# cram9030/continuum-robot

Hardware: AMD Instinct MI355X
Metric: beam-element-steps/s (higher is better)
Workload: dtype f64

## Files before the change

### continuum-robot_amd/csrc/crb_lean.h

```cpp
#pragma once
#include <hip/hip_runtime.h>

#include "crb_blocked.h"
#include "crb_generic.h"

namespace crb {

template <typename T>
struct LeanRec {
    static constexpr int N = sizeof(T) == 8 ? 10 : 12;
    static constexpr int V = 16 / sizeof(T);
};
template <typename T>
__host__ __device__ constexpr size_t lean_lds_bytes(int NT, int lognw) {
    return sizeof(T) * (size_t(NT + 1) * LeanRec<T>::N * (lognw == 1 ? 2 : 1) +
                        (sizeof(T) == 4 ? 4 : 3) * size_t(NT + 1) * size_t(lognw > 1 ? lognw - 1 : 0));
}

__device__ __forceinline__ double dpp_from_lower(double x) {
    int lo = __double2loint(x), hi = __double2hiint(x);
    lo = __builtin_amdgcn_mov_dpp(lo, 0x138, 0xf, 0xf, true);
    hi = __builtin_amdgcn_mov_dpp(hi, 0x138, 0xf, 0xf, true);
    return __hiloint2double(hi, lo);
}
__device__ __forceinline__ double dpp_from_higher(double x) {
    int lo = __double2loint(x), hi = __double2hiint(x);
    lo = __builtin_amdgcn_mov_dpp(lo, 0x130, 0xf, 0xf, true);
    hi = __builtin_amdgcn_mov_dpp(hi, 0x130, 0xf, 0xf, true);
    return __hiloint2double(hi, lo);
}
__device__ __forceinline__ float dpp_from_lower(float x) {
    return __int_as_float(__builtin_amdgcn_mov_dpp(__float_as_int(x), 0x138, 0xf, 0xf, true));
}
__device__ __forceinline__ float dpp_from_higher(float x) {
    return __int_as_float(__builtin_amdgcn_mov_dpp(__float_as_int(x), 0x130, 0xf, 0xf, true));
}
constexpr int LEAN_DPP_MAX = 4;
constexpr int P_FORCE = 0, P_XCHG = 2, P_L1 = -1, P_TAIL = 1, P_FIN = -1;
constexpr int P32_L1 = 3, P32_TAIL = 3, P32_FIN = 0;
#define CRB_SETPRIO(v) do { if ((v) >= 0) __builtin_amdgcn_s_setprio((v) < 0 ? 0 : (v)); } while (0)
template <typename T, int D>
__device__ __forceinline__ T lane_lower(T x, int lane) {
    if (D <= LEAN_DPP_MAX) {
#pragma unroll
        for (int i = 0; i < D; ++i) x = dpp_from_lower(x);
        return x;
    }
    return __shfl(x, lane - D, 64);
}
template <typename T, int D>
__device__ __forceinline__ T lane_higher(T x, int lane) {
    if (D <= LEAN_DPP_MAX) {
#pragma unroll
        for (int i = 0; i < D; ++i) x = dpp_from_higher(x);
        return x;
    }
    return __shfl(x, lane + D, 64);
}

template <typename T, int LV, int LOGNW, bool ISOLATE = false, bool RECB = false>
__device__ __forceinline__ void lean_reduce_tail(const SolveCoef<T, LV>& cf, T* ldsB, int t, int lane, int j, int S,
                                                 bool valid, T r[3], T a[3]) {
    constexpr int NW = 1 << LOGNW, NT = 64 << LOGNW, NULLT = NT;
    auto thread_of = [](int jj) { return ((jj & (NW - 1)) << 6) | (jj >> LOGNW); };
    T rlo[3], rhi[3];
#pragma unroll
    for (int l = 1; l < LV; ++l) {
        if (l < LOGNW) {
            if (l == 1) CRB_SETPRIO(sizeof(T) == 4 ? P32_L1 : P_L1);
            const int st = 1 << l;
            const int tl = (valid && j - st >= 0) ? thread_of(j - st) : NULLT;
            const int th = (valid && j + st < S) ? thread_of(j + st) : NULLT;
            if constexpr (RECB) {
                typedef T rec4 __attribute__((ext_vector_type(4)));
                rec4* buf = reinterpret_cast<rec4*>(ldsB) + size_t(l - 1) * (NT + 1);
                buf[t] = rec4{r[0], r[1], r[2], T(0)};
                __syncthreads();
                const rec4 lo = buf[tl], hi = buf[th];
#pragma unroll
                for (int c = 0; c < 3; ++c) { rlo[c] = lo[c]; rhi[c] = hi[c]; }
            } else {
                T* buf = ldsB + size_t(l - 1) * 3 * (NT + 1);
                buf[t] = r[0]; buf[(NT + 1) + t] = r[1]; buf[2 * (NT + 1) + t] = r[2];
                __syncthreads();
#pragma unroll
                for (int c = 0; c < 3; ++c) { rlo[c] = buf[c * (NT + 1) + tl]; rhi[c] = buf[c * (NT + 1) + th]; }
            }
        } else {
            if (l == LOGNW) CRB_SETPRIO(sizeof(T) == 4 ? P32_TAIL : P_TAIL);
#pragma unroll
            for (int c = 0; c < 3; ++c) {
                switch (l - LOGNW) {
                    case 0: rlo[c] = lane_lower<T, 1>(r[c], lane); rhi[c] = lane_higher<T, 1>(r[c], lane); break;
                    case 1: rlo[c] = lane_lower<T, 2>(r[c], lane); rhi[c] = lane_higher<T, 2>(r[c], lane); break;
                    case 2: rlo[c] = lane_lower<T, 4>(r[c], lane); rhi[c] = lane_higher<T, 4>(r[c], lane); break;
                    case 3: rlo[c] = lane_lower<T, 8>(r[c], lane); rhi[c] = lane_higher<T, 8>(r[c], lane); break;
                    case 4: rlo[c] = lane_lower<T, 16>(r[c], lane); rhi[c] = lane_higher<T, 16>(r[c], lane); break;
                    default: rlo[c] = lane_lower<T, 32>(r[c], lane); rhi[c] = lane_higher<T, 32>(r[c], lane); break;
                }
            }
            if (ISOLATE) {
                const int st = 1 << l;
                const bool lo_ok = valid && j - st >= 0, hi_ok = valid && j + st < S;
#pragma unroll
                for (int c = 0; c < 3; ++c) { rlo[c] = lo_ok ? rlo[c] : T(0); rhi[c] = hi_ok ? rhi[c] : T(0); }
            }
        }
        pcr_apply_level<T>(cf.lv[l], rlo, rhi, r);
    }
    CRB_SETPRIO(sizeof(T) == 4 ? P32_FIN : P_FIN);
    pcr_apply_final<T>(cf.fin, r, a);
}

template <typename T, int LV, int LOGNW, int EM>
__device__ __forceinline__ void lean_rhs(const ElemCoef<T>& ec, T dragc, bool corrected, const SolveCoef<T, LV>& cf, T* lds3, int t,
                                         int lane, int j, int S, bool valid, const T sq[3], const T sv[3], const T uadd[3], T a[3]) {
    constexpr int NW = 1 << LOGNW, NT = 64 << LOGNW, NULLT = NT;
    T* const ldsQ = lds3;
    T* const ldsA = lds3 + 3 * size_t(NT + 1);
    T* const ldsB = lds3 + 9 * size_t(NT + 1);
    auto thread_of = [](int jj) { return ((jj & (NW - 1)) << 6) | (jj >> LOGNW); };
    const int t_l1 = (valid && j >= 1) ? thread_of(j - 1) : NULLT;
    const int t_r1 = (valid && j + 1 < S) ? thread_of(j + 1) : NULLT;
    const int t_r2 = (valid && j + 2 < S) ? thread_of(j + 2) : NULLT;
    T qL[3];
    if (LOGNW == 0) {
#pragma unroll
        for (int c = 0; c < 3; ++c) qL[c] = lane_lower<T, 1>(sq[c], lane);
    } else {
#pragma unroll
        for (int c = 0; c < 3; ++c) ldsQ[size_t(c) * (NT + 1) + t] = sq[c];
        __syncthreads();
#pragma unroll
        for (int c = 0; c < 3; ++c) qL[c] = ldsQ[size_t(c) * (NT + 1) + t_l1];
    }
    T fl[3], fr[3];
    if (EM == EM_NONLINEAR) elem_force_nonlinear<T>(ec.c, qL, sq, false, fl, fr);
    else if (EM == EM_LINEAR) elem_force_linear<T>(ec.c, qL, sq, fl, fr);
    else elem_force<T>(ec, qL, sq, corrected, fl, fr);
    T pp[3];
#pragma unroll
    for (int c = 0; c < 3; ++c) pp[c] = uadd[c] - fr[c];
    pp[1] += drag_force<T>(dragc, sv[1]);
    T r[3], rlo[3], rhi[3];
    if (LOGNW == 0) {
#pragma unroll
        for (int c = 0; c < 3; ++c) {
            r[c] = pp[c] - lane_higher<T, 1>(fl[c], lane);
            rlo[c] = lane_lower<T, 1>(r[c], lane);
            rhi[c] = lane_higher<T, 1>(r[c], lane);
        }
    } else {
        auto col = [&](int k, int th) -> T& { return ldsA[size_t(k) * (NT + 1) + th]; };
#pragma unroll
        for (int c = 0; c < 3; ++c) { col(c, t) = pp[c]; col(3 + c, t) = fl[c]; }
        __syncthreads();
#pragma unroll
        for (int c = 0; c < 3; ++c) {
            rlo[c] = col(c, t_l1) - fl[c];
            r[c] = pp[c] - col(3 + c, t_r1);
            rhi[c] = col(c, t_r1) - col(3 + c, t_r2);
        }
    }
    pcr_apply_level<T>(cf.lv[0], rlo, rhi, r);
    lean_reduce_tail<T, LV, LOGNW>(cf, ldsB, t, lane, j, S, valid, r, a);
}

constexpr int BLK_STRIP_PAD = 4;
constexpr int BLK_STRIP_W = BLK_STRIP_PAD + BLK_LANES + BLK_STRIP_PAD;
__host__ __device__ constexpr size_t blk_lds_bytes(int ls) {
    return size_t(blk_sep_vals(ls) + 1) / 2 * 2 * BLK_LANES * sizeof(double) + size_t(4) * 3 * BLK_STRIP_W * sizeof(double);
}
template <typename T, int LS, int EM, typename KPT>
__device__ __forceinline__ void lean_blocked_body(KPT kp) {
    static_assert(sizeof(T) == 8, "the blocked stepper is fp64");
    static_assert(LS == 3 && (1 << (LS - 1)) == BLK_STRIP_PAD, "the strip carries the third separator level, stride 4");
    constexpr int NP = BLK_NPL, NV = blk_sep_vals(LS), NV2 = (NV + 1) / 2;
    constexpr bool REGROUP = EM == EM_NONLINEAR && !CRB_LITERAL_POLY;
#if defined(__HIP_DEVICE_COMPILE__)
    typedef const __attribute__((address_space(4))) SlotConst<T>* CS;
#define CRB_BFRESH(ptr) asm volatile("" : "+s"(ptr))
#else
    typedef const SlotConst<T>* CS;
#define CRB_BFRESH(ptr) (void)(ptr)
#endif
    typedef T rec4 __attribute__((ext_vector_type(4)));
    typedef T pair2 __attribute__((ext_vector_type(2)));
    KParams<T> p = *(const KParams<T>*)(kp);
    extern __shared__ __attribute__((aligned(16))) unsigned char crb_smem[];
    pair2* const sepL = reinterpret_cast<pair2*>(crb_smem);
    T* const strips = reinterpret_cast<T*>(sepL + NV2 * 64);
    const int t = threadIdx.x, lane = t & 63;
    const int wave = __builtin_amdgcn_readfirstlane(t >> 6);
    {
        const T* src = p.blocked + BU_N;
        for (int i = t; i < NV2 * 64; i += 256) {
            const int v = 2 * (i >> 6), l = i & 63;
            sepL[i] = pair2{src[size_t(v) * 64 + l], v + 1 < NV ? src[size_t(v + 1) * 64 + l] : T(0)};
        }
        for (int i = t; i < 4 * 3 * BLK_STRIP_W; i += 256) {
            const int k = i % BLK_STRIP_W;
            if (k < BLK_STRIP_PAD || k >= BLK_STRIP_PAD + BLK_LANES) strips[i] = T(0);
        }
    }
#if defined(__HIP_DEVICE_COMPILE__)
    typedef volatile __attribute__((address_space(3))) T* SP;
#else
    typedef volatile T* SP;
#endif
    const SP strip = (SP)(strips + wave * 3 * BLK_STRIP_W + BLK_STRIP_PAD + lane);
    T tab[BLK_TAB_REGS];
#pragma unroll
    for (int i = 0; i < BLK_TAB_REGS; ++i) tab[i] = p.blocked[blk_tab_index(i, lane)];
    const T cD2[3] = {blk_bc_copy<BU_D2>(tab), blk_bc_copy<BU_D2 + 2>(tab), blk_bc_copy<BU_D2 + 4>(tab)};
    const T cD1[3] = {blk_bc_copy<BU_U1>(tab), blk_bc_copy<BU_D1 + 2>(tab), blk_bc_copy<BU_D1 + 4>(tab)};
    const T cD0[3] = {blk_bc_copy<BU_U0>(tab), blk_bc_copy<BU_D0 + 2>(tab), blk_bc_copy<BU_D0 + 4>(tab)};
    __syncthreads();
    const int n_groups = (p.B + 3) / 4;
    for (int grp = blockIdx.x; grp < n_groups; grp += gridDim.x) {
        CRB_BFRESH(kp);
        p = *(const KParams<T>*)(kp);
        const int beam = grp * 4 + wave;
        if (beam >= p.B) continue;
        const size_t plane = size_t(p.n_node) * 4;
        const size_t xoff = size_t(beam) * 2 * plane + size_t(NP * lane + p.off) * 4;
        T xq[NP][3], xv[NP][3];
#pragma unroll
        for (int k = 0; k < NP; ++k) {
            const rec4 a = *reinterpret_cast<const rec4*>(p.x + xoff + 4 * k), b = *reinterpret_cast<const rec4*>(p.x + xoff + plane + 4 * k);
#pragma unroll
            for (int c = 0; c < 3; ++c) { xq[k][c] = a[c]; xv[k][c] = b[c]; }
        }
        T amp = T(0);
        int kimp = -1;
        if (p.amp) {
            const int js = p.imp_node_b ? p.imp_node_b[beam] - p.off : p.imp_slot;
            if (js >= 0 && js < BLK_S) {
                kimp = js & (NP - 1);
                if (lane == js / NP) amp = p.amp[beam];
            }
        }
        T qL[3];
#pragma unroll
        for (int c = 0; c < 3; ++c) qL[c] = dpp_from_lower(xq[NP - 1][c]);
        const T dt = T(p.dt), hdt = T(0.5 * p.dt), dt6 = T(p.dt / 6.0);
        double tc = p.t0;
        T accq[NP][3], accv[NP][3], sq[NP][3], sv[NP][3];
        for (int step = 0; step < p.n_steps; ++step) {
            double t_half, t_full;
            {
                KPT ks = kp;
                CRB_BFRESH(ks);
                const double hstep = (*(const KParams<T>*)(ks)).dt;
                t_half = __dadd_rn(tc, 0.5 * hstep);
                t_full = __dadd_rn(tc, hstep);
            }
#pragma unroll
            for (int k = 0; k < NP; ++k)
#pragma unroll
                for (int c = 0; c < 3; ++c) { sq[k][c] = xq[k][c]; sv[k][c] = xv[k][c]; }
#pragma unroll
            for (int s = 0; s < 4; ++s) {
                KPT ks = kp;
                CRB_BFRESH(ks);
                const KParams<T>& q = *(const KParams<T>*)(ks);
                const double ts = (s == 0) ? tc : ((s == 3) ? t_full : t_half);
                const bool imp_on = ts < q.duration;
                const T w = (s == 0 || s == 3) ? T(1) : T(2);
                const T cs = (s == 2) ? dt : hdt;
                const CS SC = (CS)q.slot;
                T ec[6];
#pragma unroll
                for (int i = 0; i < 6; ++i) ec[i] = SC->elem.c[i];
                const T drag_all = SC->drag;
                const T dragc = (q.flags & 1u) ? drag_all : T(0);
                T qn3[3], qLn[3];
#pragma unroll
                for (int k = 0; k < NP; ++k)
#pragma unroll
                    for (int c = 0; c < 3; ++c) accq[k][c] = (s == 0) ? sv[k][c] : accq[k][c] + w * sv[k][c];
#pragma unroll
                for (int c = 0; c < 3; ++c) {
                    qn3[c] = (s == 3) ? (xq[NP - 1][c] + dt6 * accq[NP - 1][c]) : (xq[NP - 1][c] + cs * sv[NP - 1][c]);
                    qLn[c] = dpp_from_lower(qn3[c]);
                }
                CRB_SETPRIO(P_FORCE);
                T fl[NP][3], r[NP][3];
                T fr[NP][3];
                T f2[NP], cW[NP];
#pragma unroll
                for (int k = 0; k < NP; ++k) {
                    if constexpr (REGROUP) {
                        const ElemForceRegrouped<T> e = elem_force_nonlinear_regrouped<T>(ec, k ? sq[k - 1] : qL, sq[k]);
                        f2[k] = e.f2; cW[k] = ec[1] * e.W;
                        fl[k][1] = e.f3; fr[k][1] = -e.f3; fl[k][2] = e.m_left; fr[k][2] = e.m_right;
                    } else if (EM == EM_NONLINEAR) elem_force_nonlinear<T>(ec, k ? sq[k - 1] : qL, sq[k], false, fl[k], fr[k]);
                    else elem_force_linear<T>(ec, k ? sq[k - 1] : qL, sq[k], fl[k], fr[k]);
                }
                if constexpr (REGROUP) {
                    fl[0][0] = cW[0] - f2[0];
#pragma unroll
                    for (int k = 0; k + 1 < NP; ++k) fr[k][0] = f2[k] - f2[k + 1];
                    fr[NP - 1][0] = dpp_from_higher(fl[0][0]);
                }
                {
                    const int kon = imp_on ? kimp : -1, dof = q.imp_dof;
#if defined(__HIP_DEVICE_COMPILE__)
#pragma unroll
                    for (int k = 0; k < NP; ++k)
                        asm volatile(
                            "s_cmp_lg_u32 %[kon], %[k]\n\t"
                            "s_cbranch_scc1 2f\n\t"
                            "s_cmp_lg_u32 %[dof], 0\n\t"
                            "s_cbranch_scc1 0f\n\t"
                            "v_add_f64 %[f0], %[f0], -%[amp]\n"
                            "0:\n\t"
                            "s_cmp_lg_u32 %[dof], 1\n\t"
                            "s_cbranch_scc1 1f\n\t"
                            "v_add_f64 %[f1], %[f1], -%[amp]\n"
                            "1:\n\t"
                            "s_cmp_lg_u32 %[dof], 2\n\t"
                            "s_cbranch_scc1 2f\n\t"
                            "v_add_f64 %[f2], %[f2], -%[amp]\n"
                            "2:"
                            : [f0] "+v"(fr[k][0]), [f1] "+v"(fr[k][1]), [f2] "+v"(fr[k][2])
                            : [kon] "s"(kon), [dof] "s"(dof), [amp] "v"(amp), [k] "n"(k)
                            : "scc");
#else
                    for (int k = 0; k < NP; ++k)
                        for (int c = 0; c < 3; ++c) fr[k][c] -= (kon == k && c == dof) ? amp : T(0);
#endif
                }
                CRB_SETPRIO(P_TAIL);
#pragma unroll
                for (int c = 0; c < 3; ++c) {
                    if (REGROUP && c == 0) {
#pragma unroll
                        for (int k = 0; k < NP; ++k) r[k][0] = (k + 1 < NP) ? (-fr[k][0] - cW[k + 1]) : (-f2[k] - fr[k][0]);
                        continue;
                    }
                    const T flR = dpp_from_higher(fl[0][c]);
#pragma unroll
                    for (int k = 0; k < NP; ++k) {
                        T h = -fr[k][c];
                        if (c == 1) h += drag_force<T>(dragc, sv[k][1]);
                        r[k][c] = h - ((k + 1 < NP) ? fl[k + 1][c] : flR);
                    }
                }
                T y[3][3], z1[3], z2[3], g[3], y0R[3];
                int li = lane;
                T cf0[PCR_LEVEL_VALS];
                asm volatile("" : "+v"(li) : "v"(r[0][0]));
#pragma unroll
                for (int i = 0; i < PCR_LEVEL_VALS; i += 2) {
                    const pair2 e = sepL[(i / 2) * 64 + li];
                    cf0[i] = e[0]; cf0[i + 1] = e[1];
                }
#pragma unroll
                for (int c = 0; c < 3; ++c) { z1[c] = r[1][c]; z2[c] = r[2][c]; g[c] = r[NP - 1][c]; }
                blk_bc_sub_mul<BU_L1>(tab, r[0], z1);
                blk_bc_sub_mul<BU_L2>(tab, z1, z2);
                y[2][0] = cD2[0] * z2[0];
                y[2][1] = cD2[1] * z2[2]; blk_bc_fma<BU_D2 + 1>(tab, z2[1], y[2][1]);
                y[2][2] = cD2[2] * z2[2]; blk_bc_fma<BU_D2 + 3>(tab, z2[1], y[2][2]);
                y[1][0] = -(cD1[0] * y[2][0]); blk_bc_fma<BU_D1>(tab, z1[0], y[1][0]);
                y[1][1] = cD1[1] * z1[2]; blk_bc_fma<BU_D1 + 1>(tab, z1[1], y[1][1]);
                y[1][2] = cD1[2] * z1[2]; blk_bc_fma<BU_D1 + 3>(tab, z1[1], y[1][2]);
                blk_bc_fnma<BU_U1 + 1>(tab, y[2][1], y[1][1]); blk_bc_fnma<BU_U1 + 2>(tab, y[2][2], y[1][1]);
                blk_bc_fnma<BU_U1 + 3>(tab, y[2][1], y[1][2]); blk_bc_fnma<BU_U1 + 4>(tab, y[2][2], y[1][2]);
                y[0][0] = -(cD0[0] * y[1][0]); blk_bc_fma<BU_D0>(tab, r[0][0], y[0][0]);
                y[0][1] = cD0[1] * r[0][2]; blk_bc_fma<BU_D0 + 1>(tab, r[0][1], y[0][1]);
                y[0][2] = cD0[2] * r[0][2]; blk_bc_fma<BU_D0 + 3>(tab, r[0][1], y[0][2]);
                blk_bc_fnma<BU_U0 + 1>(tab, y[1][1], y[0][1]); blk_bc_fnma<BU_U0 + 2>(tab, y[1][2], y[0][1]);
                blk_bc_fnma<BU_U0 + 3>(tab, y[1][1], y[0][2]); blk_bc_fnma<BU_U0 + 4>(tab, y[1][2], y[0][2]);
#pragma unroll
                for (int c = 0; c < 3; ++c) y0R[c] = dpp_from_higher(y[0][c]);
                blk_bc_sub_mul<BU_AS>(tab, y[2], g);
                blk_bc_sub_mul<BU_CS>(tab, y0R, g);
#pragma unroll
                for (int l = 0; l < LS; ++l) {
                    asm volatile("" : "+v"(li) : "v"(g[0]));
                    T cf[PCR_LEVEL_VALS];
#pragma unroll
                    for (int i = 0; i < PCR_LEVEL_VALS; i += 2) {
                        const int v = l * PCR_LEVEL_VALS + i;
                        if (l == 0) { cf[i] = cf0[i]; cf[i + 1] = cf0[i + 1]; continue; }
                        const pair2 e = sepL[(v / 2) * 64 + li];
                        cf[i] = e[0]; cf[i + 1] = e[1];
                    }
                    T glo[3], ghi[3];
                    if (l == 2) {
#pragma unroll
                        for (int c = 0; c < 3; ++c) strip[c * BLK_STRIP_W] = g[c];
#pragma unroll
                        for (int c = 0; c < 3; ++c) { glo[c] = strip[c * BLK_STRIP_W - 4]; ghi[c] = strip[c * BLK_STRIP_W + 4]; }
                    } else if (l == 1) {
#pragma unroll
                        for (int c = 0; c < 3; ++c) { glo[c] = lane_lower<T, 2>(g[c], lane); ghi[c] = lane_higher<T, 2>(g[c], lane); }
                    } else {
#pragma unroll
                        for (int c = 0; c < 3; ++c) { glo[c] = lane_lower<T, 1>(g[c], lane); ghi[c] = lane_higher<T, 1>(g[c], lane); }
                    }
                    pcr_apply_level<T>(cf, glo, ghi, g);
                }
                asm volatile("" : "+v"(li) : "v"(g[0]));
                T fin[6], xs[3], xsL[3];
#pragma unroll
                for (int i = 0; i < 6; i += 2) {
                    const int v = LS * PCR_LEVEL_VALS + i;
                    const pair2 e = sepL[(v / 2) * 64 + li];
                    fin[i] = e[0]; fin[i + 1] = e[1];
                }
                pcr_apply_final<T>(fin, g, xs);
#pragma unroll
                for (int c = 0; c < 3; ++c) xsL[c] = dpp_from_lower(xs[c]);
                T a[NP][3];
#pragma unroll
                for (int k = 0; k < NP - 1; ++k)
#pragma unroll
                    for (int c = 0; c < 3; ++c) a[k][c] = y[k][c];
                static_assert(NP == 4, "three interior nodes, written out: the table offsets are template arguments");
                blk_bc_sub_mul<BU_WL>(tab, xsL, a[0]);
                blk_bc_sub_mul<BU_WR>(tab, xs, a[0]);
                blk_bc_sub_mul<BU_WL + BLK_PACK>(tab, xsL, a[1]);
                blk_bc_sub_mul<BU_WR + BLK_PACK>(tab, xs, a[1]);
                blk_bc_sub_mul<BU_WL + 2 * BLK_PACK>(tab, xsL, a[2]);
                blk_bc_sub_mul<BU_WR + 2 * BLK_PACK>(tab, xs, a[2]);
#pragma unroll
                for (int c = 0; c < 3; ++c) a[NP - 1][c] = xs[c];
#pragma unroll
                for (int k = 0; k < NP; ++k)
#pragma unroll
                    for (int c = 0; c < 3; ++c) {
                        accv[k][c] = (s == 0) ? a[k][c] : accv[k][c] + w * a[k][c];
                        if (k == NP - 1) sq[k][c] = qn3[c];
                        else sq[k][c] = (s == 3) ? (xq[k][c] + dt6 * accq[k][c]) : (xq[k][c] + cs * sv[k][c]);
                        sv[k][c] = (s == 3) ? (xv[k][c] + dt6 * accv[k][c]) : (xv[k][c] + cs * a[k][c]);
                    }
#pragma unroll
                for (int c = 0; c < 3; ++c) qL[c] = qLn[c];
            }
#pragma unroll
            for (int k = 0; k < NP; ++k)
#pragma unroll
                for (int c = 0; c < 3; ++c) { xq[k][c] = sq[k][c]; xv[k][c] = sv[k][c]; }
            tc = t_full;
            KPT kr_ = kp;
            CRB_BFRESH(kr_);
            const KParams<T>& pr = *(const KParams<T>*)(kr_);
            if (pr.rec_out && (step + 1) % pr.rec_every == 0) {
                const size_t kr = size_t((step + 1) / pr.rec_every - 1);
                if (pr.rec_slot == REC_ALL_SLOTS) {
                    T* snap = pr.rec_out + kr * size_t(pr.B) * 2 * plane + xoff;
#pragma unroll
                    for (int k = 0; k < NP; ++k) {
                        *reinterpret_cast<rec4*>(snap + 4 * k) = rec4{xq[k][0], xq[k][1], xq[k][2], T(0)};
                        *reinterpret_cast<rec4*>(snap + plane + 4 * k) = rec4{xv[k][0], xv[k][1], xv[k][2], T(0)};
                    }
                } else if (pr.rec_slot >= 0 && lane == pr.rec_slot / NP) {
                    const int kk = pr.rec_slot & (NP - 1);
                    T val = xq[0][0];
#pragma unroll
                    for (int k = 0; k < NP; ++k)
#pragma unroll
                        for (int c = 0; c < 6; ++c)
                            val = (k == kk && c == pr.rec_comp) ? (c < 3 ? xq[k][c] : xv[k][c - 3]) : val;
                    pr.rec_out[size_t(beam) * pr.rec_n + kr] = val;
                }
            }
        }
        CRB_BFRESH(kp);
        p = *(const KParams<T>*)(kp);
        bool bad = false;
#pragma unroll
        for (int k = 0; k < NP; ++k) {
            *reinterpret_cast<rec4*>(p.x + xoff + 4 * k) = rec4{xq[k][0], xq[k][1], xq[k][2], T(0)};
            *reinterpret_cast<rec4*>(p.x + xoff + plane + 4 * k) = rec4{xv[k][0], xv[k][1], xv[k][2], T(0)};
#pragma unroll
            for (int c = 0; c < 3; ++c) bad = bad || !isfinite(xq[k][c]) || !isfinite(xv[k][c]);
        }
        if (p.status && bad) atomicCAS(p.status + beam, 0, p.status_value);
    }
#undef CRB_BFRESH
}

__host__ __device__ constexpr int lean_minw_f64(int lv, int lognw, bool grav) { return (grav && lv >= 5 && lognw == 0) ? 1 : 2; }
template <typename T, int LV, int LOGNW, bool GRAV, int EM, bool HELD = false, bool PACK = false, bool FB = false, int NPL = 1>
__global__ void __launch_bounds__(64 << LOGNW, FB ? 1 : ((sizeof(T) == 4 && LOGNW <= 2) ? ((LV <= 4 && !GRAV && !HELD) ? 4 : 3) : lean_minw_f64(LV, LOGNW, GRAV)))
crb_step_lean_kernel(const KParams<T> p_formal) {
#if defined(__HIP_DEVICE_COMPILE__)
    typedef const __attribute__((address_space(4))) KParams<T>* KP;
    KP kp = (KP)__builtin_amdgcn_kernarg_segment_ptr();
    (void)p_formal;
#define CRB_FRESH(ptr) asm volatile("" : "+s"(ptr))
#define CRB_PARAMS(ptr) (*(const KParams<T>*)(ptr))
#else
    const KParams<T>* kp = &p_formal;
#define CRB_FRESH(ptr) (void)(ptr)
#define CRB_PARAMS(ptr) (*(ptr))
#endif
    if constexpr (NPL > 1) {
        static_assert(NPL == BLK_NPL && LOGNW == 2 && !GRAV && !HELD && !PACK && !FB, "the blocked form is the plain 256-slot stepper");
        lean_blocked_body<T, LV, EM>(kp);
        return;
    }
    KParams<T> p = CRB_PARAMS(kp);
    static_assert(!PACK || LOGNW == 0, "packed beams live inside one wave");
    static_assert(!FB || (PACK && !HELD), "the feedback form is the packed one-wave stepper");
    static_assert(LV >= 1, "lean stepper needs at least one reduction level");
    constexpr int NW = 1 << LOGNW, NT = 64 << LOGNW, RN = LeanRec<T>::N;
    constexpr int NULLT = NT;
    constexpr bool SOA = sizeof(T) == 8;
    constexpr bool RECB = sizeof(T) == 4;
    auto recA = [](T* base, int th, int k) -> T& { return SOA ? base[size_t(k) * (NT + 1) + th] : base[size_t(th) * RN + k]; };
    extern __shared__ __attribute__((aligned(16))) unsigned char crb_smem[];
    T* const ldsA = reinterpret_cast<T*>(crb_smem);
    T* const ldsB = ldsA + size_t(NT + 1) * RN * (LOGNW == 1 ? 2 : 1);

    const int t = threadIdx.x, lane = t & 63, wave = t >> 6;
    const int S = p.S;
    const int pg = PACK ? lane / S : 0;
    const int j = PACK ? lane - pg * S : ((lane << LOGNW) | wave);
    const bool has_slot = PACK ? (pg < p.G) : (j < S);
    auto thread_of = [](int jj) { return ((jj & (NW - 1)) << 6) | (jj >> LOGNW); };
    const int t_l1 = (has_slot && j >= 1) ? thread_of(j - 1) : NULLT;
    const int t_r1 = (has_slot && j + 1 < S) ? thread_of(j + 1) : NULLT;
    if (LOGNW > 0 && t == 0) {
#pragma unroll
        for (int k = 0; k < RN; ++k) {
            recA(ldsA, NULLT, k) = T(0);
            if (LOGNW == 1) recA(ldsA + size_t(NT + 1) * RN, NULLT, k) = T(0);
        }
#pragma unroll
        for (int l = 1; l < LOGNW; ++l)
#pragma unroll
            for (int c = 0; c < (RECB ? 4 : 3); ++c)
                ldsB[RECB ? (size_t(l - 1) * (NT + 1) + NULLT) * 4 + c : (size_t(l - 1) * 3 + c) * (NT + 1) + NULLT] = T(0);
    }

    const bool shared_tables = p.slot_stride == 0 && p.lv_stride == 0 && p.fin_stride == 0;
    ElemCoef<T> ec;
    T dragc = T(0);
    SolveCoef<T, LV> cf;
    T hm_own = T(0), hm_left = T(0);
    auto load_tables = [&](int beam) {
        if (has_slot) {
            const SlotConst<T>* st = p.slot + size_t(beam) * p.slot_stride;
            const SlotConst<T>& sc = st[j];
            ec = sc.elem;
            dragc = (p.flags & 1u) ? sc.drag : T(0);
            if (GRAV) { hm_own = sc.half_mass; hm_left = j >= 1 ? st[j - 1].half_mass : T(0); }
#pragma unroll
            for (int l = 0; l < LV; ++l) {
                const T* src = p.pcr_levels + size_t(beam) * p.lv_stride + (size_t(l) * size_t(S) + size_t(j)) * PCR_LEVEL_VALS;
#pragma unroll
                for (int k = 0; k < PCR_LEVEL_VALS; ++k) cf.lv[l][k] = src[k];
            }
#pragma unroll
            for (int k = 0; k < 5; ++k) cf.fin[k] = p.pcr_final[size_t(beam) * p.fin_stride + size_t(j) * PCR_FINAL_VALS + k];
        } else {
            ec = padding_slot<T>().elem;
#pragma unroll
            for (int l = 0; l < LV; ++l)
#pragma unroll
                for (int k = 0; k < PCR_LEVEL_VALS; ++k) cf.lv[l][k] = T(0);
#pragma unroll
            for (int k = 0; k < 5; ++k) cf.fin[k] = T(0);
        }
    };
    if (shared_tables) load_tables(0);
    const int fb_n = FB ? p.n_red : 0, fb_n2 = 2 * fb_n, fb_n2p = fb_padded(fb_n2), fb_G = FB ? p.G : 0;
    T* const fbx = reinterpret_cast<T*>(crb_smem);
    T* const fbK = fbx + size_t(fb_G) * fb_n2p;
    T* const fbu = fbK + size_t(fb_n2p) * fb_n;
    const bool fb_mfma = FB && fb_on_matrix_cores(fb_G, fb_n);
    T fb_af[FBM_MT][FBM_KS];
    if (FB) {
        for (int idx = t; idx < fb_n * fb_n2; idx += NT) {
            const int i = idx / fb_n2, k = idx - i * fb_n2;
            fbK[size_t(k) * fb_n + i] = p.fb_gain[idx];
        }
        for (int idx = t; idx < (fb_n2p - fb_n2) * fb_n; idx += NT) fbK[size_t(fb_n2) * fb_n + idx] = T(0);
        for (int idx = t; idx < fb_G * (fb_n2p - fb_n2); idx += NT)
            fbx[size_t(idx / (fb_n2p - fb_n2)) * fb_n2p + fb_n2 + idx % (fb_n2p - fb_n2)] = T(0);
        __syncthreads();
        if (fb_mfma) fbm_gain_fragments<T>(fb_af, fbK, fb_n, fb_n2p, lane);
    }
    const bool corrected = (p.flags & 4u) != 0;
    const T dt = T(p.dt), hdt = T(0.5 * p.dt), dt6 = T(p.dt / 6.0);
    const size_t plane = size_t(p.n_node) * 4;
    const int n_groups = PACK ? (p.B + p.G - 1) / p.G : p.B;

    constexpr bool PREFETCH = !PACK && !FB;
    T nq[3] = {T(0), T(0), T(0)}, nv[3] = {T(0), T(0), T(0)}, namp = T(0);
    bool have_next = false;
    int mask_bits = 7;
    if (PREFETCH && shared_tables && has_slot) {
        const SlotConst<T>& sc0 = p.slot[j];
// ... 501 lines not shown
```

### continuum-robot_amd/csrc/crb_math.h

```cpp
#pragma once
#include <math.h>
#include <stdint.h>

#if defined(__HIPCC__)
#define CRB_HD __host__ __device__ __forceinline__
#else
#define CRB_HD inline
#endif

namespace crb {

enum : int { KIND_NONE = 0, KIND_LINEAR = 1, KIND_NONLINEAR = 2 };

template <typename T>
struct ElemCoef {
    T c[6];
    int32_t kind;
    int32_t pad;
};

template <typename T>
CRB_HD void elem_coef_build(ElemCoef<T>& e, int kind, double L, double E, double I, double A) {
    const double EA = E * A, EI = E * I;
    e.kind = kind;
// ... 5 lines not shown
        e.c[3] = T(4 * EI / L);
        e.c[4] = T(2 * EI / L);
        e.c[5] = T(0);
    } else if (kind == KIND_NONLINEAR) {
        const double iL2 = 1.0 / (L * L), tenth_iL3 = 0.1 / (L * L * L);
        e.c[0] = T(L);
        e.c[1] = T(EA * iL2);
        e.c[2] = T(EA * tenth_iL3);
        e.c[3] = T(20.0 * EI * tenth_iL3);
        e.c[4] = T(0.5 * EA * iL2);
        e.c[5] = T(EI * iL2);
    } else {
        for (int i = 0; i < 6; ++i) e.c[i] = T(0);
    }
}

template <typename T>
CRB_HD void elem_force_linear(const T* c, const T ql[3], const T qr[3], T fl[3], T fr[3]) {
    const T du = ql[0] - qr[0];
    const T dw = ql[1] - qr[1];
    const T fa = c[0] * du;
    const T fw = c[1] * dw - c[2] * (ql[2] + qr[2]);
    const T m0 = -c[2] * dw;
    fl[0] = fa;
    fl[1] = fw;
    fl[2] = m0 + c[3] * ql[2] + c[4] * qr[2];
    fr[0] = -fa;
    fr[1] = -fw;
    fr[2] = m0 + c[4] * ql[2] + c[3] * qr[2];
}

template <typename T>
CRB_HD T plus_remainder(T base, double c, T ww) {
    return c == 0.0 ? base : base + T(c) * ww;
}

template <typename T>
CRB_HD void elem_force_nonlinear_literal(const T* c, const T ql[3], const T qr[3], bool corrected, T fl[3], T fr[3]) {
    const T L = c[0], A = c[1], D = c[2], iL2 = c[3], tenth_iL3 = c[4];
    const T u1 = ql[0], w1 = ql[1], u2 = qr[0], w2 = qr[1];
    const T a = ql[2] * L, b = qr[2] * L;
    const T du = u1 - u2, dw = w1 - w2;
    const T ww = w1 * w2, dw2 = dw * dw;
    const T a2 = a * a, b2 = b * b, ab = a * b;
    const T Ldu = L * du;

    const T T0 = T(0.6) * dw - T(0.05) * (a + b);
    const T P = a * (T(0.0666666666666665) * a - T(0.0166666666666667) * b - T(0.05) * dw) -
                b * (T(0.0166666666666667) * a - T(0.0666666666666667) * b + T(0.05) * dw);
    const T f2 = A * iL2 * (P - Ldu + dw * T0);
    const T f1 = corrected ? -f2 : A * iL2 * (L * u1 - P - (u2 + dw) * T0);

    const T Qa = plus_remainder<T>(T(3.8571428571413) * dw2, 2.0 * 3.8571428571413 - 7.7142857142826, ww);
    const T Qb = plus_remainder<T>(T(3.857142857143) * dw2, 2.0 * 3.857142857143 - 7.71428571428601, ww);
    const T Cw = dw * plus_remainder<T>(T(10.2857142857147) * dw2, 3.0 * 10.2857142857147 - 30.857142857144, ww);
    const T P3 = T(0.0357142857143344) * (a2 * a + b2 * b) - T(0.107142857143003) * ab * (a + b) +
                 T(1.28571428571433) * (a2 + b2) * dw + Ldu * (a + b) - a * Qa - b * Qb - T(12.0) * Ldu * dw + Cw;
    const T f3 = tenth_iL3 * (A * P3 + D * (T(120.0) * dw - T(60.0) * (a + b)));

    const T Q4 = plus_remainder<T>(T(0.128571428571433) * dw2, 2.0 * 0.128571428571433 - 0.257142857142867, ww);
    const T C4 = dw * plus_remainder<T>(T(0.128571428571377) * dw2, 3.0 * 0.128571428571377 - 0.38571428571413, ww);
    const T P4 = T(0.0285714285714391) * a2 * a - T(0.0107142857142861) * a2 * b + T(0.0107142857142719) * a2 * dw +
                 T(0.00714285714286444) * a * b2 - T(0.0214285714286007) * ab * dw - T(0.133333333333333) * a * Ldu +
                 a * Q4 - T(0.00357142857143344) * b2 * b - T(0.0107142857142719) * b2 * dw +
                 T(0.0333333333333333) * b * Ldu + T(0.1) * Ldu * dw - C4;
    const T f4 = iL2 * (A * P4 + D * (T(4.0) * a + T(2.0) * b - T(6.0) * dw));

    const T Q6 = plus_remainder<T>(T(0.128571428571428) * dw2, 2.0 * 0.128571428571428 - 0.257142857142856, ww);
    const T C6 = dw * plus_remainder<T>(T(0.128571428571433) * dw2, 3.0 * 0.128571428571433 - 0.3857142857143, ww);
    const T P6 = -T(0.00357142857143344) * a2 * a + T(0.00714285714286356) * a2 * b - T(0.0107142857143003) * a2 * dw -
                 T(0.0107142857142932) * a * b2 - T(0.021428571428558) * ab * dw + T(0.0333333333333333) * a * Ldu +
                 T(0.0285714285714271) * b2 * b + T(0.0107142857142932) * b2 * dw - T(0.133333333333333) * b * Ldu +
                 b * Q6 + T(0.1) * Ldu * dw - C6;
    const T f6 = iL2 * (A * P6 + D * (T(2.0) * a + T(4.0) * b - T(6.0) * dw));

    fl[0] = f1;
    fl[1] = f3;
    fl[2] = f4;
    fr[0] = f2;
    fr[1] = -f3;
    fr[2] = f6;
}

template <typename T>
CRB_HD void elem_force_nonlinear_sym(const T* c, const T ql[3], const T qr[3], bool corrected, T fl[3], T fr[3]) {
    const T L = c[0], cA1 = c[1], cA3 = c[2], cD3 = c[3], cA4 = c[4], cD4 = c[5];
    const T u1 = ql[0], u2 = qr[0];
    const T a = ql[2] * L, b = qr[2] * L;
    const T du = u1 - u2, dw = ql[1] - qr[1];
    const T s = a + b, d = a - b, p = a * b;
    const T s2 = s * s, dw2 = dw * dw, Ldu = L * du;

    const T T0 = T(0.6) * dw - T(0.05) * s;
    const T P = s * (T(1.0 / 15.0) * s - T(0.05) * dw) - T(1.0 / 6.0) * p;
    const T f2 = cA1 * (P - Ldu + dw * T0);
    const T f1 = corrected ? -f2 : cA1 * (L * u1 - P - (u2 + dw) * T0);

    const T P3 = s * (T(1.0 / 28.0) * (s2 - T(6.0) * p) + Ldu - T(27.0 / 7.0) * dw2) +
                 dw * (T(9.0 / 7.0) * (s2 - T(2.0) * p) - T(12.0) * Ldu + T(72.0 / 7.0) * dw2);
    const T g = T(3.0) * s - T(6.0) * dw;
    const T f3 = cA3 * P3 - cD3 * g;

    const T S = s * (T(1.0 / 40.0) * s2 - T(11.0 / 140.0) * p - T(0.1) * Ldu + T(9.0 / 70.0) * dw2) +
                dw * (T(0.2) * Ldu - T(3.0 / 70.0) * p - T(9.0 / 35.0) * dw2);
    const T R = T(9.0 / 280.0) * s2 - T(0.05) * p + T(3.0 / 140.0) * (s * dw) - T(1.0 / 6.0) * Ldu +
                T(9.0 / 70.0) * dw2;
    const T X = cA4 * S + cD4 * g;
    const T Y = d * (cA4 * R + cD4);

    fl[0] = f1;
    fl[1] = f3;
    fl[2] = X + Y;
    fr[0] = f2;
    fr[1] = -f3;
    fr[2] = X - Y;
}

template <typename T>
struct ElemForceRegrouped {
    T f2, W, f3, m_left, m_right;
};
template <typename T>
CRB_HD ElemForceRegrouped<T> elem_force_nonlinear_regrouped(const T* c, const T ql[3], const T qr[3]) {
    const T L = c[0], cA1 = c[1], cA3 = c[2], cD3 = c[3], cA4 = c[4], cD4 = c[5];
    const T u1 = ql[0], u2 = qr[0];
    const T a = ql[2] * L, b = qr[2] * L;
    const T du = u1 - u2, dw = ql[1] - qr[1];
    const T s = a + b, d = a - b, p = a * b;
    const T s2 = s * s, dw2 = dw * dw, Ldu = L * du, sdw = s * dw;

    T E = T(1.0 / 15.0) * s2 - Ldu;
    E = E - T(0.1) * sdw;
    E = E - T(1.0 / 6.0) * p;
    E = E + T(0.6) * dw2;
    T LT = L + T(0.05) * s;
    LT = LT - T(0.6) * dw;

    const T P3 = s * (T(1.0 / 28.0) * (s2 - T(6.0) * p) + Ldu - T(27.0 / 7.0) * dw2) +
                 dw * (T(9.0 / 7.0) * (s2 - T(2.0) * p) - T(12.0) * Ldu + T(72.0 / 7.0) * dw2);
    const T g = T(3.0) * s - T(6.0) * dw;
    const T S = s * (T(1.0 / 40.0) * s2 - T(11.0 / 140.0) * p - T(0.1) * Ldu + T(9.0 / 70.0) * dw2) +
                dw * (T(0.2) * Ldu - T(3.0 / 70.0) * p - T(9.0 / 35.0) * dw2);
    const T R = T(9.0 / 280.0) * s2 - T(0.05) * p + T(3.0 / 140.0) * sdw - T(1.0 / 6.0) * Ldu + T(9.0 / 70.0) * dw2;
    const T X = cA4 * S + cD4 * g;
    const T Y = d * (cA4 * R + cD4);

    ElemForceRegrouped<T> o;
    o.f2 = cA1 * E;
    o.W = u2 * LT;
    o.f3 = cA3 * P3 - cD3 * g;
    o.m_left = X + Y;
    o.m_right = X - Y;
    return o;
}

#ifndef CRB_LITERAL_POLY
#define CRB_LITERAL_POLY 0
#endif
template <typename T>
CRB_HD void elem_force_nonlinear(const T* c, const T ql[3], const T qr[3], bool corrected, T fl[3], T fr[3]) {
#if CRB_LITERAL_POLY
    const T iL2 = T(1) / (c[0] * c[0]);
    const T lit[5] = {c[0], c[1] / iL2, c[5] / iL2, iL2, T(0.1) * iL2 / c[0]};
    elem_force_nonlinear_literal<T>(lit, ql, qr, corrected, fl, fr);
#else
    elem_force_nonlinear_sym<T>(c, ql, qr, corrected, fl, fr);
#endif
}

template <typename T>
CRB_HD void elem_force(const ElemCoef<T>& e, const T ql[3], const T qr[3], bool corrected, T fl[3], T fr[3]) {
    if (e.kind == KIND_NONLINEAR) {
        elem_force_nonlinear<T>(e.c, ql, qr, corrected, fl, fr);
    } else if (e.kind == KIND_LINEAR) {
        elem_force_linear<T>(e.c, ql, qr, fl, fr);
    } else {
        fl[0] = fl[1] = fl[2] = fr[0] = fr[1] = fr[2] = T(0);
    }
}

CRB_HD void crb_sincos(double x, double* s, double* c) {
#if defined(__HIP_DEVICE_COMPILE__)
    ::sincos(x, s, c);
#else
    *s = sin(x);
    *c = cos(x);
#endif
}
CRB_HD void crb_sincos(float x, float* s, float* c) {
#if defined(__HIP_DEVICE_COMPILE__)
    ::sincosf(x, s, c);
#else
    *s = sinf(x);
    *c = cosf(x);
#endif
}

template <typename T>
CRB_HD void gravity_segment(T phi, T gx, T gy, T half_mass, T out[2]) {
    T s, c;
    crb_sincos(phi, &s, &c);
    out[0] = (c * gx + s * gy) * half_mass;
    out[1] = (c * gy - s * gx) * half_mass;
}

CRB_HD double crb_abs(double v) { return __builtin_fabs(v); }
CRB_HD float crb_abs(float v) { return __builtin_fabsf(v); }
template <typename T>
CRB_HD T drag_force(T coef, T v) {
    return -coef * v * crb_abs(v);
}

struct NodeBlocks {
    double a_ax, b_ax, c_ax;
    double A[4], B[4], C[4];
};

CRB_HD void mass_add_as_right_elem(NodeBlocks& n, double L, double rhoA) {
    const double m = rhoA * L / 420.0;
    n.b_ax += 140.0 * m;
    n.c_ax += 70.0 * m;
    n.B[0] += 156.0 * m;
    n.B[1] += -22.0 * L * m;
    n.B[2] += -22.0 * L * m;
    n.B[3] += 4.0 * L * L * m;
    n.C[0] += 54.0 * m;
    n.C[1] += 13.0 * L * m;
    n.C[2] += -13.0 * L * m;
    n.C[3] += -3.0 * L * L * m;
}
CRB_HD void mass_add_as_left_elem(NodeBlocks& n, double L, double rhoA, bool has_left_node) {
    const double m = rhoA * L / 420.0;
    n.b_ax += 140.0 * m;
    n.B[0] += 156.0 * m;
    n.B[1] += 22.0 * L * m;
    n.B[2] += 22.0 * L * m;
    n.B[3] += 4.0 * L * L * m;
    if (has_left_node) {
        n.a_ax += 70.0 * m;
        n.A[0] += 54.0 * m;
        n.A[1] += -13.0 * L * m;
        n.A[2] += 13.0 * L * m;
        n.A[3] += -3.0 * L * L * m;
    }
}

CRB_HD void stiff_add_as_right_elem(NodeBlocks& n, double L, double EA, double EI, double alpha, bool axial_12) {
    const double c0 = alpha * EA / L, c1 = alpha * 12 * EI / (L * L * L), c2 = alpha * 6 * EI / (L * L), c3 = alpha * 4 * EI / L,
                 c4 = alpha * 2 * EI / L;
    n.b_ax += c0;
    if (axial_12) n.c_ax += -c0;
    n.B[0] += c1; n.B[1] += -c2; n.B[2] += -c2; n.B[3] += c3;
    n.C[0] += -c1; n.C[1] += -c2; n.C[2] += c2; n.C[3] += c4;
}
CRB_HD void stiff_add_as_left_elem(NodeBlocks& n, double L, double EA, double EI, double alpha, bool has_left_node) {
    const double c0 = alpha * EA / L, c1 = alpha * 12 * EI / (L * L * L), c2 = alpha * 6 * EI / (L * L), c3 = alpha * 4 * EI / L,
                 c4 = alpha * 2 * EI / L;
    n.b_ax += c0;
    n.B[0] += c1; n.B[1] += c2; n.B[2] += c2; n.B[3] += c3;
    if (has_left_node) {
        n.a_ax += -c0;
        n.A[0] += -c1; n.A[1] += c2; n.A[2] += -c2; n.A[3] += c4;
    }
}

template <typename T>
CRB_HD void elem_linear_coefs(const T* c, int kind, T out[5]) {
    if (kind == KIND_NONLINEAR) {
        const T L = c[0];
        out[0] = c[1] * L;
        out[1] = T(6) * c[3];
        out[2] = T(6) * c[5];
        out[3] = T(4) * c[5] * L;
        out[4] = T(2) * c[5] * L;
    } else {
        for (int i = 0; i < 5; ++i) out[i] = c[i];
    }
}

CRB_HD void mass_apply_masks(NodeBlocks& n, bool fu, bool fw, bool fp, bool lu, bool lw, bool lp, bool ru, bool rw,
                             bool rp) {
    if (!fu) { n.a_ax = 0; n.c_ax = 0; n.b_ax = 1; }
    if (!lu) n.a_ax = 0;
    if (!ru) n.c_ax = 0;
    const bool fr[2] = {fw, fp}, lf[2] = {lw, lp}, rf[2] = {rw, rp};
    for (int r = 0; r < 2; ++r)
        for (int cc = 0; cc < 2; ++cc) {
            if (!fr[r] || !lf[cc]) n.A[2 * r + cc] = 0;
            if (!fr[r] || !rf[cc]) n.C[2 * r + cc] = 0;
            if (!fr[r] || !fr[cc]) n.B[2 * r + cc] = (r == cc && !fr[r]) ? 1.0 : 0.0;
        }
}

CRB_HD void inv2(const double M[4], double R[4]) {
    const double det = M[0] * M[3] - M[1] * M[2];
    const double id = 1.0 / det;
    R[0] = M[3] * id;
    R[1] = -M[1] * id;
    R[2] = -M[2] * id;
    R[3] = M[0] * id;
}
CRB_HD void mul2(const double X[4], const double Y[4], double R[4]) {
    R[0] = X[0] * Y[0] + X[1] * Y[2];
    R[1] = X[0] * Y[1] + X[1] * Y[3];
    R[2] = X[2] * Y[0] + X[3] * Y[2];
    R[3] = X[2] * Y[1] + X[3] * Y[3];
// ... 185 lines not shown
```

Measured before the change: 71.17 billion.

## Use chord-variable element force and closed-form RK4 position updates in blocked stepper

Adds a chord-based reformulation of the regrouped nonlinear element force, built on e = s - 2dw, to cut the polynomial operation count. It also restructures the RK4 position update so stage positions come from precomputed dt^2-weighted acceleration sums. This drops the per-stage accq accumulation and most stage-velocity recomputation, keeping only the c==1 velocity that is still needed. Both are on by default through macros. The rearranged arithmetic changes floating-point rounding relative to the literal RK4 scheme.

```diff
diff --git a/continuum-robot_amd/csrc/crb_lean.h b/continuum-robot_amd/csrc/crb_lean.h
--- a/continuum-robot_amd/csrc/crb_lean.h
+++ b/continuum-robot_amd/csrc/crb_lean.h
@@ -166,6 +166,12 @@
     lean_reduce_tail<T, LV, LOGNW>(cf, ldsB, t, lane, j, S, valid, r, a);
 }
 
+#ifndef CRB_BLK_CHORD
+#define CRB_BLK_CHORD 1
+#endif
+#ifndef CRB_BLK_RK4_POS
+#define CRB_BLK_RK4_POS 1
+#endif
 constexpr int BLK_STRIP_PAD = 4;
 constexpr int BLK_STRIP_W = BLK_STRIP_PAD + BLK_LANES + BLK_STRIP_PAD;
 __host__ __device__ constexpr size_t blk_lds_bytes(int ls) {
@@ -177,6 +183,7 @@
     static_assert(LS == 3 && (1 << (LS - 1)) == BLK_STRIP_PAD, "the strip carries the third separator level, stride 4");
     constexpr int NP = BLK_NPL, NV = blk_sep_vals(LS), NV2 = (NV + 1) / 2;
     constexpr bool REGROUP = EM == EM_NONLINEAR && !CRB_LITERAL_POLY;
+    constexpr bool CHORD = CRB_BLK_CHORD, RKPOS = CRB_BLK_RK4_POS;
 #if defined(__HIP_DEVICE_COMPILE__)
     typedef const __attribute__((address_space(4))) SlotConst<T>* CS;
 #define CRB_BFRESH(ptr) asm volatile("" : "+s"(ptr))
@@ -244,8 +251,11 @@
 #pragma unroll
         for (int c = 0; c < 3; ++c) qL[c] = dpp_from_lower(xq[NP - 1][c]);
         const T dt = T(p.dt), hdt = T(0.5 * p.dt), dt6 = T(p.dt / 6.0);
+        [[maybe_unused]] const T c6 = T(p.dt * p.dt / 6.0), c4 = T(0.25 * p.dt * p.dt), c2 = T(0.5 * p.dt * p.dt);
         double tc = p.t0;
-        T accq[NP][3], accv[NP][3], sq[NP][3], sv[NP][3];
+        [[maybe_unused]] T accq[NP][3], accv[NP][3];
+        T sq[NP][3], sv[NP][3];
+        [[maybe_unused]] Rk4Pos<T> rk[NP][3];
         for (int step = 0; step < p.n_steps; ++step) {
             double t_half, t_full;
             {
@@ -274,15 +284,27 @@
                 for (int i = 0; i < 6; ++i) ec[i] = SC->elem.c[i];
                 const T drag_all = SC->drag;
                 const T dragc = (q.flags & 1u) ? drag_all : T(0);
-                T qn3[3], qLn[3];
-#pragma unroll
-                for (int k = 0; k < NP; ++k)
-#pragma unroll
-                    for (int c = 0; c < 3; ++c) accq[k][c] = (s == 0) ? sv[k][c] : accq[k][c] + w * sv[k][c];
-#pragma unroll
-                for (int c = 0; c < 3; ++c) {
-                    qn3[c] = (s == 3) ? (xq[NP - 1][c] + dt6 * accq[NP - 1][c]) : (xq[NP - 1][c] + cs * sv[NP - 1][c]);
-                    qLn[c] = dpp_from_lower(qn3[c]);
+                [[maybe_unused]] T qn3[3];
+                T qLn[3];
+                if constexpr (RKPOS) {
+                    if (s == 0) {
+#pragma unroll
+                        for (int k = 0; k < NP; ++k)
+#pragma unroll
+                            for (int c = 0; c < 3; ++c) rk4_begin<T>(rk[k][c], xq[k][c], xv[k][c], hdt, dt);
+                    }
+#pragma unroll
+                    for (int c = 0; c < 3; ++c) qLn[c] = dpp_from_lower(rk[NP - 1][c].next);
+                } else {
+#pragma unroll
+                    for (int k = 0; k < NP; ++k)
+#pragma unroll
+                        for (int c = 0; c < 3; ++c) accq[k][c] = (s == 0) ? sv[k][c] : accq[k][c] + w * sv[k][c];
+#pragma unroll
+                    for (int c = 0; c < 3; ++c) {
+                        qn3[c] = (s == 3) ? (xq[NP - 1][c] + dt6 * accq[NP - 1][c]) : (xq[NP - 1][c] + cs * sv[NP - 1][c]);
+                        qLn[c] = dpp_from_lower(qn3[c]);
+                    }
                 }
                 CRB_SETPRIO(P_FORCE);
                 T fl[NP][3], r[NP][3];
@@ -291,7 +313,8 @@
 #pragma unroll
                 for (int k = 0; k < NP; ++k) {
                     if constexpr (REGROUP) {
-                        const ElemForceRegrouped<T> e = elem_force_nonlinear_regrouped<T>(ec, k ? sq[k - 1] : qL, sq[k]);
+                        const ElemForceRegrouped<T> e = CHORD ? elem_force_nonlinear_chord<T>(ec, k ? sq[k - 1] : qL, sq[k])
+                                                              : elem_force_nonlinear_regrouped<T>(ec, k ? sq[k - 1] : qL, sq[k]);
                         f2[k] = e.f2; cW[k] = ec[1] * e.W;
                         fl[k][1] = e.f3; fr[k][1] = -e.f3; fl[k][2] = e.m_left; fr[k][2] = e.m_right;
                     } else if (EM == EM_NONLINEAR) elem_force_nonlinear<T>(ec, k ? sq[k - 1] : qL, sq[k], false, fl[k], fr[k]);
@@ -432,10 +455,19 @@
                 for (int k = 0; k < NP; ++k)
 #pragma unroll
                     for (int c = 0; c < 3; ++c) {
-                        accv[k][c] = (s == 0) ? a[k][c] : accv[k][c] + w * a[k][c];
-                        if (k == NP - 1) sq[k][c] = qn3[c];
-                        else sq[k][c] = (s == 3) ? (xq[k][c] + dt6 * accq[k][c]) : (xq[k][c] + cs * sv[k][c]);
-                        sv[k][c] = (s == 3) ? (xv[k][c] + dt6 * accv[k][c]) : (xv[k][c] + cs * a[k][c]);
+                        if constexpr (RKPOS) {
+                            sq[k][c] = rk[k][c].next;
+                            if (s == 0) rk4_end0<T>(rk[k][c], a[k][c], c6, c4);
+                            else if (s == 1) rk4_end1<T>(rk[k][c], a[k][c], c6, c2);
+                            else if (s == 2) rk4_end2<T>(rk[k][c], a[k][c], c6);
+                            else xv[k][c] = rk4_end3<T>(rk[k][c], xv[k][c], a[k][c], dt6);
+                            if (c == 1 && s < 3) sv[k][1] = rk4_stage_velocity<T>(xv[k][1], cs, a[k][1]);
+                        } else {
+                            accv[k][c] = (s == 0) ? a[k][c] : accv[k][c] + w * a[k][c];
+                            if (k == NP - 1) sq[k][c] = qn3[c];
+                            else sq[k][c] = (s == 3) ? (xq[k][c] + dt6 * accq[k][c]) : (xq[k][c] + cs * sv[k][c]);
+                            sv[k][c] = (s == 3) ? (xv[k][c] + dt6 * accv[k][c]) : (xv[k][c] + cs * a[k][c]);
+                        }
                     }
 #pragma unroll
                 for (int c = 0; c < 3; ++c) qL[c] = qLn[c];
@@ -443,7 +475,10 @@
 #pragma unroll
             for (int k = 0; k < NP; ++k)
 #pragma unroll
-                for (int c = 0; c < 3; ++c) { xq[k][c] = sq[k][c]; xv[k][c] = sv[k][c]; }
+                for (int c = 0; c < 3; ++c) {
+                    xq[k][c] = sq[k][c];
+                    if (!RKPOS) xv[k][c] = sv[k][c];
+                }
             tc = t_full;
             KPT kr_ = kp;
             CRB_BFRESH(kr_);
diff --git a/continuum-robot_amd/csrc/crb_math.h b/continuum-robot_amd/csrc/crb_math.h
--- a/continuum-robot_amd/csrc/crb_math.h
+++ b/continuum-robot_amd/csrc/crb_math.h
@@ -181,6 +181,89 @@
     o.m_left = X + Y;
     o.m_right = X - Y;
     return o;
+}
+
+template <typename T>
+CRB_HD ElemForceRegrouped<T> elem_force_nonlinear_chord(const T* c, const T ql[3], const T qr[3]) {
+    const T L = c[0], cA1 = c[1], cA3 = c[2], cD3 = c[3], cA4 = c[4], cD4 = c[5];
+    const T u2 = qr[0];
+    const T a = ql[2] * L, b = qr[2] * L;
+    const T du = ql[0] - u2, dw = ql[1] - qr[1];
+    const T s = a + b, d = a - b;
+    const T e = s - T(2.0) * dw;
+    const T e2 = e * e, d2 = d * d, dw2 = dw * dw, U = L * du;
+
+    T E = T(0.5) * dw2 - U;
+    E = E + T(1.0 / 24.0) * d2;
+    E = E + T(1.0 / 40.0) * e2;
+    T LT = L + T(0.05) * e;
+    LT = LT - T(0.5) * dw;
+
+    T P3e = U + T(3.0 / 56.0) * d2;
+    P3e = P3e - T(1.5) * dw2;
+    P3e = P3e - T(1.0 / 56.0) * e2;
+    T P3w = T(0.75) * d2 - T(10.0) * U;
+    P3w = P3w + T(5.0) * dw2;
+    P3w = P3w + T(15.0 / 28.0) * e2;
+    const T P3 = e * P3e + dw * P3w;
+    const T g = T(3.0) * e;
+    T Se = T(11.0 / 560.0) * d2 - T(0.1) * U;
+    Se = Se + T(0.15) * dw2;
+    Se = Se + T(3.0 / 560.0) * e2;
+    const T Sw = T(0.05) * d2 + T(3.0 / 140.0) * e2;
+    const T S = e * Se + dw * Sw;
+    T R = T(1.0 / 80.0) * d2 - T(1.0 / 6.0) * U;
+    R = R + T(11.0 / 560.0) * e2;
+    R = R + dw * (T(0.25) * dw + T(0.1) * e);
+    const T X = cA4 * S + cD4 * g;
+    const T Y = d * (cA4 * R + cD4);
+
+    ElemForceRegrouped<T> o;
+    o.f2 = cA1 * E;
+    o.W = u2 * LT;
+    o.f3 = cA3 * P3 - cD3 * g;
+    o.m_left = X + Y;
+    o.m_right = X - Y;
+    return o;
+}
+
+template <typename T>
+struct Rk4Pos {
+    T next;
+    T full;
+    T sum;
+    T accv;
+};
+template <typename T>
+CRB_HD void rk4_begin(Rk4Pos<T>& r, T q, T v, T hdt, T dt) {
+    r.next = q + hdt * v;
+    r.full = q + dt * v;
+}
+template <typename T>
+CRB_HD void rk4_end0(Rk4Pos<T>& r, T a, T c6, T c4) {
+    r.accv = a;
+    r.sum = r.full + c6 * a;
+    r.next = r.next + c4 * a;
+}
+template <typename T>
+CRB_HD void rk4_end1(Rk4Pos<T>& r, T a, T c6, T c2) {
+    r.accv = r.accv + T(2) * a;
+    r.sum = r.sum + c6 * a;
+    r.full = r.full + c2 * a;
+    r.next = r.full;
+}
+template <typename T>
+CRB_HD void rk4_end2(Rk4Pos<T>& r, T a, T c6) {
+    r.accv = r.accv + T(2) * a;
+    r.next = r.sum + c6 * a;
+}
+template <typename T>
+CRB_HD T rk4_end3(const Rk4Pos<T>& r, T v, T a, T dt6) {
+    return v + dt6 * (r.accv + a);
+}
+template <typename T>
+CRB_HD T rk4_stage_velocity(T v, T cs, T a) {
+    return v + cs * a;
 }
 
 #ifndef CRB_LITERAL_POLY
```

Result: faster. 75.24 billion (median of 6 runs) (+5.7%).
